# ktncktnc/diffusion-forcing-transformer

Hardware: AMD Instinct MI355X
Metric: denoised latent frames/sec, DFoT RE10K 8f & 200f rollout @1/2/4/8 GPU (higher is better)
Workload: dtype bf16

## Files before the change

diffusion-forcing-transformer_amd/backbone.py:

```python
from __future__ import annotations

import ctypes as C
import math
from typing import Dict, Optional, Sequence, Tuple

import torch
from torch import nn

from . import capi, ops
from .engine_module import EngineModule, _Node, _get

_FOURIER_BUFFERS = ("noise_level_pos_embedding.timesteps.freqs", "noise_level_pos_embedding.timesteps.phases")


class UViTModule(EngineModule):
    _family = "uvit"

    def _new_tensor(self, name: str, shape: Tuple[int, ...]) -> torch.Tensor:
        t = torch.zeros(shape, dtype=torch.float32)
        return t if name in _FOURIER_BUFFERS else nn.Parameter(t)

    def _tensors(self) -> Dict[str, torch.Tensor]:
        return self._engine_tensors()

# ... 91 lines not shown
        c.eps = 1e-6
        if int(_get(cfg, "patch_size", 2)) != 2:
            raise ValueError("only patch_size=2 is supported")
        self._ccfg = c
        self._build_tree()
        self._cond_key = None
        self._cond_refs = None
        self._cond_gen = None
        self._cond_flag = None
        self.cond_cache_stats = {"builds": 0, "identity_hits": 0, "content_hits": 0}
        self._train_names = None
        self._trainer = None
        self._trainer_sig = None
        self.live_frames = None
        self.fresh_frames = None
        self._fresh_key = None
        self._train_stamp = 0
        self._dropout_generator: Optional[torch.Generator] = None

    def _after_reserve(self) -> None:
        self._cond_key = None

    def forward(self, x: torch.Tensor, noise_levels: torch.Tensor, external_cond: Optional[torch.Tensor] = None,
                external_cond_mask: Optional[torch.Tensor] = None) -> torch.Tensor:
        assert external_cond is not None, "External condition (camera pose) is required for U-ViT3DPose model."
        if self._op_key is None:
            self._op_key = ops.register_model(self)
        if torch.is_grad_enabled() and (x.requires_grad or any(p.requires_grad for p in self.parameters())):
            if self._train_names is None:
                self._train_names = [n for n, _ in self.named_parameters()]
# ... 130 lines not shown
            self._cond_refs = (external_cond, external_cond_mask)
            self._cond_gen = self.reserve_generation
        out = torch.empty_like(xf)
        live = self.live_frames
        if live is not None:
            if tuple(live.shape) != (b, self.temporal_length) or live.dtype != torch.uint8 or not live.is_contiguous():
                raise ValueError(f"live_frames must be a contiguous uint8 tensor of shape {(b, self.temporal_length)}")
            capi.require_device(dev, live_frames=live)
        fresh = self.fresh_frames
        if fresh is not None:
            if tuple(fresh.shape) != (b, self.temporal_length) or fresh.dtype != torch.uint8 or not fresh.is_contiguous():
                raise ValueError(f"fresh_frames must be a contiguous uint8 tensor of shape {(b, self.temporal_length)}")
            capi.require_device(dev, fresh_frames=fresh)
            if key != self._fresh_key:
                fresh = None
        capi.check(capi.lib.dfot_uvit_forward_cached_masks(self._handle, capi.ptr(xf, torch.float32, "x"),
                                                           capi.ptr(kf, torch.float32, "noise_levels"), capi.ptr(out), b,
                                                           capi.ptr(live, torch.uint8, "live_frames"),
                                                           capi.ptr(fresh, torch.uint8, "fresh_frames"), capi.stream_ptr()))
        self._fresh_key = key
        return out.to(x.dtype)
```

diffusion-forcing-transformer_amd/capi.py:

```python
from __future__ import annotations

import ctypes as C
import os

_HERE = os.path.dirname(os.path.abspath(__file__))
LIB_PATH = os.environ.get("DFOT_LIB", os.path.join(_HERE, "libdfot_hip.so"))

OK, ERR_ARG, ERR_SHAPE, ERR_HIP, ERR_STATE, ERR_NAME = range(6)


class DfotError(RuntimeError):
    def __init__(self, code: int, message: str):
        super().__init__(f"libdfot_hip error {code}: {message}")
        self.code = code


class UViTConfig(C.Structure):
    _fields_ = [
        ("channels", C.c_int32 * 4), ("emb_channels", C.c_int32), ("num_updown_blocks", C.c_int32 * 3),
        ("num_mid_blocks", C.c_int32), ("num_heads", C.c_int32), ("in_channels", C.c_int32),
        ("resolution", C.c_int32), ("max_tokens", C.c_int32), ("cond_dim", C.c_int32), ("noise_dim", C.c_int32),
        ("rope_theta", C.c_float), ("eps", C.c_float),
    ]

# ... 61 lines not shown
    "dfot_uvit_num_params": (_I, [_P]),
    "dfot_uvit_param_name": (C.c_char_p, [_P, _I]),
    "dfot_uvit_param_shape": (_I, [_P, _I, C.POINTER(_L), C.POINTER(_I)]),
    "dfot_uvit_load_weight": (_I, [_P, C.c_char_p, _P, C.POINTER(_L), _I, _P]),
    "dfot_uvit_finalize": (_I, [_P, _P]),
    "dfot_uvit_reserve": (_I, [_P, _I]),
    "dfot_uvit_workspace_bytes": (C.c_size_t, [_P]),
    "dfot_uvit_set_option": (_I, [_P, C.c_char_p, _I]),
    "dfot_uvit_query": (_I, [_P, C.c_char_p, C.POINTER(C.c_double)]),
    "dfot_uvit_attn_timing": (_I, [_P, C.POINTER(C.c_double), C.POINTER(_L)]),
    "dfot_uvit_forward": (_I, [_P, _P, _P, _P, _P, _P, _I, _P]),
    "dfot_uvit_set_conditions": (_I, [_P, _P, _P, _I, _P]),
    "dfot_uvit_forward_cached": (_I, [_P, _P, _P, _P, _I, _P]),
    "dfot_uvit_forward_cached_live": (_I, [_P, _P, _P, _P, _I, _P, _P]),
    "dfot_uvit_forward_cached_masks": (_I, [_P, _P, _P, _P, _I, _P, _P, _P]),
    "dfot_uvit_read_tap": (_I, [_P, C.c_char_p, _P, C.c_size_t, _P]),
    "dfot_uvit3d_create": (_I, [C.POINTER(UViT3DConfig), C.POINTER(_P)]),
    "dfot_uvit3d_config_bytes": (_L, []),
    "dfot_uvit3d_forward": (_I, [_P, _P, _P, _P, _P, _P, _I, _P]),
    "dfot_uvit3d_forward_live": (_I, [_P, _P, _P, _P, _P, _P, _I, _P, _P]),
    "dfot_op_gn_film_silu": (_I, [_P, _P, _P, _P, _P, _P, _P, _P, _I, _I, _I, _I, _P]),
    "dfot_op_rms_film": (_I, [_P, _P, _P, _P, _P, _P, _L, _I, _I, _I, _F, _P]),
    "dfot_dit_create": (_I, [C.POINTER(DiTConfig), C.POINTER(_P)]),
    "dfot_dit_create_f": (_I, [C.POINTER(DiTConfigF), C.POINTER(_P)]),
    "dfot_dit_destroy": (_I, [_P]),
    "dfot_dit_num_params": (_I, [_P]),
    "dfot_dit_param_name": (C.c_char_p, [_P, _I]),
    "dfot_dit_param_shape": (_I, [_P, _I, C.POINTER(_L), C.POINTER(_I)]),
    "dfot_dit_load_weight": (_I, [_P, C.c_char_p, _P, C.POINTER(_L), _I, _P]),
    "dfot_dit_finalize": (_I, [_P, _P]),
# ... 244 lines not shown
```

diffusion-forcing-transformer_amd/csrc/kernels.h:

```cpp
#pragma once
#include "common.h"

namespace dfot {

int launch_noise_emb(const float* k, const float* freqs, const float* phases, const float* w1, const float* b1,
                     const float* w2, const float* b2, float* hidden, float* out, int bt, int ndim, int e, hipStream_t s);
int launch_uvit3d_emb(const float* k, const float* freqs, const float* phases, const float* w1, const float* b1, const float* w2,
                      const float* b2, const float* cond, const uint8_t* cond_mask, const float* a_w1, const float* a_b1,
                      const float* a_w2, const float* a_b2, float* out, int bt, int ndim, int cdim, int e, int tokens, hipStream_t s);
int launch_embed_input(const float* x, const float* w, const float* b, float* out, int bt, int res, int cin, int c0,
                       hipStream_t s);
int launch_cond_repack(const float* cond, bf16* a, int bt, int res, int cdim, int kpad, hipStream_t s);
int launch_emb_pyramid(const bf16* emb0, bf16* emb1, bf16* emb2, bf16* emb3, int bt, int r0, int e, hipStream_t s);
int launch_project_output(const float* x0, const float* w, const float* b, float* out, int bt, int res, int c0, int cout,
                          hipStream_t s, const uint8_t* live = nullptr);
int launch_gn_partial_f32(const float* x, float* partial, int bt, int pixels, int c, hipStream_t s);
int launch_gn_partial_bf16(const bf16* x, float* partial, int bt, int pixels, int c, hipStream_t s);
int launch_gn_finalize(const float* partial, float* stats, int bt, int nblk, int pixels, int c, float eps, hipStream_t s);
int gn_partial_blocks(int pixels);
int launch_gn_apply_silu(const float* x, const float* stats, const float* gamma, const float* beta, bf16* out, int bt,
                         int pixels, int c, hipStream_t s, const uint8_t* live = nullptr);
struct FilmChunk {
  const bf16* w;
  const float* b;
// ... 15 lines not shown
                    long m, int c, int rows_per_bt, int tokens, float eps, hipStream_t s, const RmsPending* pend = nullptr);
int launch_rms_film_bf16(const bf16* x, const float* w, const bf16* fcache, const float* sv, const uint8_t* cond_mask, bf16* out,
                         long m, int c, int rows_per_bt, int tokens, float eps, hipStream_t s, const RmsPending* pend = nullptr);

int launch_pool2_bf16(const float* x, bf16* out, int bt, int h, int w, int c, hipStream_t s);
int launch_pool2_bf16_bf16in(const bf16* x, bf16* out, int bt, int h, int w, int c, hipStream_t s);
int launch_sub_bf16_bf16in(const bf16* a, const float* b, bf16* out, long n, hipStream_t s, const uint8_t* live = nullptr, long frame_elems = 0);
int launch_upsample_add_bf16(const float* t, const bf16* skip, bf16* out, int bt, int h, int w, int c, hipStream_t s, const uint8_t* live = nullptr);
int launch_gn_apply_silu_bf16in(const bf16* x, const float* stats, const float* gamma, const float* beta, bf16* out, int bt, int pixels, int c,
                                hipStream_t s, const uint8_t* live = nullptr);
int launch_embed_input_bf16(const float* x, const float* w, const float* b, bf16* out, int bt, int res, int cin, int c0, hipStream_t s);
int launch_project_output_bf16(const bf16* x0, const float* w, const float* b, float* out, int bt, int res, int c0, int cout, hipStream_t s,
                               const uint8_t* live = nullptr);
int launch_sub_bf16(const float* a, const float* b, bf16* out, long n, hipStream_t s, const uint8_t* live = nullptr, long frame_elems = 0);
int launch_upsample_add(const float* t, const float* skip, float* out, int bt, int h, int w, int c, hipStream_t s, const uint8_t* live = nullptr);
int launch_ray_encode(const float* poses, float* out, int b, int t, int res, int normalized, hipStream_t s);
int launch_hg_prepare(const float* x, const float* noise, const float* qa, const float* qb, float* x_in, int batch,
                      int nfe, int tokens, long f, hipStream_t s);
int launch_ddim_compose(const float* x, const float* x_in, const float* v, const float* sa, const float* s1,
                        const float* an, const float* cn, const float* keep, const float* weight, const uint8_t* gen,
                        float* x_next, int batch, int nfe, int tokens, long f, bool weight_per_token, hipStream_t s);
int launch_ddim_noise(const float* noise, const float* sigma, const float* weight, const uint8_t* gen, float* x_next, int batch, int nfe,
                      int tokens, long f, bool weight_per_token, hipStream_t s);
int vloss_chunks(long f);
int launch_vloss(const float* x, const float* noise, const float* v, const float* a, const float* sg, const float* w,
                 float* x_pred, float* partial, float* loss, int batch, int tokens, long f, bool vspace, hipStream_t s);
int launch_wgrad_nt(const bf16* a, long lda, const bf16* b, long ldb, float* out, int m, int n, long rows, int slices, hipStream_t s, int img_h = 0,
                    int img_w = 0, int sdy = 0, int sdx = 0, int all_taps = 0);
struct WgradPlan {
  int form, slices;
// ... 80 lines not shown
```

diffusion-forcing-transformer_amd/csrc/kernels.hip:

```cpp
#include "kernels.h"
#include "dfot_hip.h"

namespace dfot {

typedef __attribute__((ext_vector_type(4))) float float4v;
typedef __attribute__((ext_vector_type(2))) float float2v;

__device__ __forceinline__ float wave_sum(float v) {
#pragma unroll
  for (int o = 32; o > 0; o >>= 1) v += __shfl_xor(v, o);
  return v;
}

template <bool FOURIER>
__global__ __launch_bounds__(256) void noise_mlp_kernel(const float* __restrict__ in, const float* __restrict__ freqs,
                                                        const float* __restrict__ phases, const float* __restrict__ w,
                                                        const float* __restrict__ b, float* __restrict__ out, int kdim,
                                                        int e) {
  const int lane = threadIdx.x & 63, wave = threadIdx.x >> 6;
  const int row = blockIdx.x * 4 + wave;
  const int bt = blockIdx.y;
  if (row >= e) return;
  float acc = 0.f;
  for (int i = lane; i < kdim; i += 64) {
// ... 1509 lines not shown
  hipLaunchKernelGGL(equal_bits_kernel<T>, dim3(grid), dim3(EQ_BLOCK), 0, s, (const T*)a, (const T*)b, n, rest, differs);
  DFOT_CHECK_HIP(hipGetLastError());
  return DFOT_OK;
}

int launch_equal_bits(const void* a, const void* b, long bytes, int* differs, hipStream_t s) {
  DFOT_REQUIRE(differs && ((uintptr_t)differs & 3) == 0, DFOT_ERR_ARG, "equal_bits: the flag is null or not 4-byte aligned");
  DFOT_REQUIRE(bytes >= 0, DFOT_ERR_ARG, "equal_bits: negative length %ld", bytes);
  if (bytes == 0) return DFOT_OK;
  DFOT_REQUIRE(a && b, DFOT_ERR_ARG, "equal_bits: null buffer");
  const uintptr_t al = (uintptr_t)a | (uintptr_t)b;
  if ((al & 15) == 0) return launch_equal_bits_t<uint4v>(a, b, bytes, differs, s);
  if ((al & 3) == 0) return launch_equal_bits_t<unsigned int>(a, b, bytes, differs, s);
  return launch_equal_bits_t<uint8_t>(a, b, bytes, differs, s);
}
}

extern "C" int dfot_op_equal_bits(const void* a, const void* b, int64_t bytes, int32_t* differs, void* stream) {
  return dfot::launch_equal_bits(a, b, (long)bytes, differs, (hipStream_t)stream);
}
```

diffusion-forcing-transformer_amd/csrc/uvit.hip:

```cpp
#include <algorithm>
#include <cmath>
#include <cstdarg>
#include <cstdlib>
#include <cstring>
#include <string>
#include <vector>

#include "dfot_hip.h"
#include "engine_device.h"
#include "gemm.h"
#include "kernels.h"

namespace dfot {

static thread_local char g_err[1024] = "";
void set_error(const char* fmt, ...) {
  va_list ap;
  va_start(ap, fmt);
  vsnprintf(g_err, sizeof(g_err), fmt, ap);
  va_end(ap);
}
const char* get_error() { return g_err; }

int tuning_flag(const char* name, int dflt) {
// ... 59 lines not shown
  int film_chunks = 0;
  uint8_t* cond_mask = nullptr;
  bool have_mask = false;
  int cond_batch = 0;
  int64_t cond_builds = 0;
  bf16 *acond = nullptr, *emb[4] = {nullptr, nullptr, nullptr, nullptr}, *s1 = nullptr, *hbf = nullptr,
       *cat = nullptr, *q = nullptr, *k = nullptr, *v = nullptr;
  AttnScratch attn_scratch;
  const float* pend_part = nullptr;
  float* out_part = nullptr;
  size_t out_part_elems = 0;
  const float* pend_bias = nullptr;
  int pend_lvl = 0, pend_c = 0, pend_slices = 2;
  long pend_m = 0;
  int last_batch = 0;
  const float* xin[4] = {nullptr, nullptr, nullptr, nullptr};
  bf16* XB[4] = {nullptr, nullptr, nullptr, nullptr};
  bool xin_bf[4] = {false, false, false, false};
  int gemm_variant = GEMM_AUTO;
  int attn_variant = 2;
  bool attn_force_safe = false;
  bool time_attn = false;
  std::vector<hipEvent_t> ev_start, ev_stop;
  size_t ev_used = 0;
};

namespace dfot {

static int add_res_block(dfot_uvit_s* h, const std::string& pre, int c, ResW* w) {
  const int e = h->E;
// ... 393 lines not shown
  g.A = h->s1; g.W = h->up_conv[l].w; g.M = bt * rr * rr; g.N = cout; g.K = 9 * cin; g.H = rr; g.Wd = rr; g.Cin = cin;
  g.zeros = h->zeros; g.bias = h->up_conv[l].b; g.out_f32 = h->tmp; g.ldo = cout;
  if (live && (rr * rr) % 256 == 0 && h->gemm_variant == GEMM_AUTO) g.live = live;
  if ((rc = conv_between_levels(h, g, s))) return rc;
  h->gn1_nblk = 0;
  if (!h->xin_bf[l]) {
    set_error("run_up: level %d stream is not in its bf16 buffer", l);
    return DFOT_ERR_STATE;
  }
  return launch_upsample_add_bf16(h->tmp, h->XB[l], h->XB[l], bt, rr, rr, cout, s, live);
}

}

static int forward_from_emb(dfot_uvit_s* h, const float* x, float* out, int batch, const uint8_t* live_frames, const uint8_t* fresh_frames,
                            hipStream_t s);

extern "C" {

const char* dfot_last_error(void) { return get_error(); }
int dfot_version(void) { return 1; }

int dfot_uvit_create(const dfot_uvit_config* cfg, dfot_uvit_t* out) {
  DFOT_REQUIRE(cfg && out, DFOT_ERR_ARG, "dfot_uvit_create: null argument");
  DFOT_REQUIRE(cfg->resolution % 16 == 0 && cfg->resolution >= 32, DFOT_ERR_SHAPE, "resolution %d must be a multiple of 16", cfg->resolution);
  DFOT_REQUIRE(cfg->emb_channels % 64 == 0, DFOT_ERR_SHAPE, "emb_channels %d must be a multiple of 64", cfg->emb_channels);
  DFOT_REQUIRE(cfg->in_channels <= 3 && cfg->cond_dim % 20 == 0, DFOT_ERR_SHAPE, "in_channels %d / cond_dim %d unsupported", cfg->in_channels, cfg->cond_dim);
  for (int l = 0; l < 4; ++l)
    DFOT_REQUIRE(cfg->channels[l] % 64 == 0, DFOT_ERR_SHAPE, "channels[%d]=%d must be a multiple of 64", l, cfg->channels[l]);
  DFOT_REQUIRE(cfg->channels[0] % 128 == 0 && cfg->channels[1] % 128 == 0, DFOT_ERR_SHAPE, "ResBlock channels must be multiples of 128");
  for (int l = 2; l < 4; ++l) {
// ... 165 lines not shown
      sv_off += (long)bt * 2 * c;
      return DFOT_OK;
    };
    for (int l = 0; l < 2; ++l) {
      for (ResW& w : h->down_res[l]) if ((rc = add(&w.fcache, &w.sv_off, w.w_film, w.b_film, w.c, l))) return rc;
      for (ResW& w : h->up_res[l]) if ((rc = add(&w.fcache, &w.sv_off, w.w_film, w.b_film, w.c, l))) return rc;
    }
    for (TrW& w : h->down_tr) if ((rc = add(&w.fcache, &w.sv_off, w.w_film, w.b_film, w.c, 2))) return rc;
    for (TrW& w : h->up_tr) if ((rc = add(&w.fcache, &w.sv_off, w.w_film, w.b_film, w.c, 2))) return rc;
    for (TrW& w : h->mid_tr) if ((rc = add(&w.fcache, &w.sv_off, w.w_film, w.b_film, w.c, 3))) return rc;
    if ((rc = h->alloc(&h->sv, (size_t)sv_off, true))) return rc;
    if ((rc = h->alloc(&h->film_table, table.size(), true))) return rc;
    DFOT_CHECK_HIP(hipMemcpy(h->film_table, table.data(), table.size() * sizeof(FilmChunk), hipMemcpyHostToDevice));
    h->film_chunks = (int)table.size();
    if ((rc = h->alloc(&h->cond_mask, (size_t)max_batch, true))) return rc;
    h->cond_batch = 0;
  }
  if ((rc = h->alloc(&h->cat, mc * 5, true))) return rc;
  if ((rc = h->alloc(&h->q, mc, true))) return rc;
  if ((rc = h->alloc(&h->k, mc, true))) return rc;
  if ((rc = h->alloc(&h->v, mc, true))) return rc;
  {
    const size_t e2 = bt * pix[2] * h->ch[2], e3 = bt * pix[3] * h->ch[3];
    h->out_part_elems = 3 * (e2 > e3 ? e2 : e3);
    if ((rc = h->alloc(&h->out_part, h->out_part_elems, true))) return rc;
  }
  {
    size_t need = 16;
    for (int b = 1; b <= max_batch; ++b)
      for (int l = 2; l < 4; ++l) need = std::max(need, attention_scratch_bytes(b, h->heads, h->T * h->r[l] * h->r[l], h->ch[l] / h->heads));
// ... 99 lines not shown
  h->cond_batch = batch;
  return DFOT_OK;
}

int dfot_uvit_forward_cached(dfot_uvit_t h, const float* x, const float* noise_levels, float* out, int batch, void* stream) {
  return dfot_uvit_forward_cached_live(h, x, noise_levels, out, batch, nullptr, stream);
}

int dfot_uvit_forward_cached_live(dfot_uvit_t h, const float* x, const float* noise_levels, float* out, int batch, const uint8_t* live_frames,
                                  void* stream) {
  return dfot_uvit_forward_cached_masks(h, x, noise_levels, out, batch, live_frames, nullptr, stream);
}

int dfot_uvit_forward_cached_masks(dfot_uvit_t h, const float* x, const float* noise_levels, float* out, int batch, const uint8_t* live_frames,
                                   const uint8_t* fresh_frames, void* stream) {
  DFOT_REQUIRE(h && x && noise_levels && out, DFOT_ERR_ARG, "forward: null argument");
  DFOT_REQUIRE(!fresh_frames || h->last_batch == batch, DFOT_ERR_STATE,
               "forward: frozen frames need the previous forward of this handle to have run the same batch (%d, now %d)", h->last_batch, batch);
  DFOT_REQUIRE(!fresh_frames || live_frames, DFOT_ERR_ARG, "forward: frozen frames must also be dead frames (live_frames is null)");
  DFOT_REQUIRE(!h->posefree, DFOT_ERR_STATE, "forward_cached: a pose-free handle (dfot_uvit3d_create) runs through dfot_uvit3d_forward");
  DFOT_REQUIRE(h->finalized, DFOT_ERR_STATE, "forward: weights not finalized");
  DFOT_REQUIRE(batch > 0 && batch == h->cond_batch, DFOT_ERR_STATE,
               "forward_cached: batch %d does not match the cached conditions (%d)", batch, h->cond_batch);
  hipStream_t s = (hipStream_t)stream;
  const dfot_uvit_config& c = h->cfg;
  const int bt = batch * h->T, e = h->E;
  int rc = 0;
  if ((rc = launch_noise_emb(noise_levels, h->ne_freqs, h->ne_phases, h->ne_w1, h->ne_b1, h->ne_w2, h->ne_b2, h->nhid,
                             h->nemb, bt, c.noise_dim, e, s)))
    return rc;
  return forward_from_emb(h, x, out, batch, live_frames, fresh_frames, s);
}

}

static int forward_from_emb(dfot_uvit_s* h, const float* x, float* out, int batch, const uint8_t* live_frames, const uint8_t* fresh_frames,
                            hipStream_t s) {
  const dfot_uvit_config& c = h->cfg;
  const int bt = batch * h->T, e = h->E;
  int rc = 0;
  if ((rc = launch_film_vec(h->film_table, h->film_chunks, h->nemb, h->sv, bt, e, s))) return rc;
  if ((rc = launch_embed_input_bf16(x, h->ein_w, h->ein_b, h->XB[0], bt, c.resolution, c.in_channels, h->ch[0], s))) return rc;
  h->gn1_nblk = 0;
  for (int l = 0; l < 4; ++l) h->xin[l] = h->X[l];
  h->xin_bf[0] = true;
  h->xin_bf[1] = h->xin_bf[2] = h->xin_bf[3] = false;

  if (fresh_frames && (h->gemm_variant != GEMM_AUTO || (h->r[2] * h->r[2]) % 512 != 0)) fresh_frames = nullptr;
  for (int l = 0; l < 2; ++l) {
    for (const ResW& w : h->down_res[l])
      if ((rc = run_res_block(h, w, l, bt, s, fresh_frames))) return rc;
    if ((rc = run_down(h, l, bt, s, fresh_frames))) return rc;
  }
  h->pend_bias = nullptr;
  for (const TrW& w : h->down_tr)
    if ((rc = run_tr_block(h, w, 2, batch, s))) return rc;
  if ((rc = flush_pending(h, s))) return rc;
  if ((rc = run_down(h, 2, bt, s))) return rc;
  for (const TrW& w : h->mid_tr)
    if ((rc = run_tr_block(h, w, 3, batch, s))) return rc;
  if ((rc = flush_pending(h, s))) return rc;
  if ((rc = run_up(h, 2, bt, s))) return rc;
  for (const TrW& w : h->up_tr)
    if ((rc = run_tr_block(h, w, 2, batch, s))) return rc;
  if ((rc = flush_pending(h, s))) return rc;
  for (int l = 1; l >= 0; --l) {
    if ((rc = run_up(h, l, bt, s, live_frames))) return rc;
// ... 16 lines not shown

int dfot_uvit3d_forward_live(dfot_uvit_t h, const float* x, const float* noise_levels, const float* external_cond,
                             const uint8_t* external_cond_mask, float* out, int batch, const uint8_t* live_frames, void* stream) {
  DFOT_REQUIRE(h && x && noise_levels && out, DFOT_ERR_ARG, "uvit3d_forward: null argument");
  DFOT_REQUIRE(h->posefree, DFOT_ERR_STATE, "uvit3d_forward: the handle is a pose model (dfot_uvit_create); call dfot_uvit_forward");
  DFOT_REQUIRE(h->finalized, DFOT_ERR_STATE, "uvit3d_forward: weights not finalized");
  DFOT_REQUIRE(batch > 0 && batch <= h->max_batch, DFOT_ERR_STATE, "uvit3d_forward: batch %d exceeds reserved %d", batch, h->max_batch);
  DFOT_REQUIRE(!external_cond || h->act_dim > 0, DFOT_ERR_ARG,
               "uvit3d_forward: external_cond given, but the model was built with cond_dim 0 (no external_cond_embedding)");
  hipStream_t s = (hipStream_t)stream;
  const uint8_t* mask = (external_cond && h->act_dropout) ? external_cond_mask : nullptr;
  int rc = launch_uvit3d_emb(noise_levels, h->ne_freqs, h->ne_phases, h->ne_w1, h->ne_b1, h->ne_w2, h->ne_b2, external_cond, mask, h->ac_w1,
                             h->ac_b1, h->ac_w2, h->ac_b2, h->nemb, batch * h->T, h->cfg.noise_dim, h->act_dim, h->E, h->T, s);
  if (rc) return rc;
  h->have_mask = false;
  return forward_from_emb(h, x, out, batch, live_frames, nullptr, s);
}

int dfot_uvit3d_forward(dfot_uvit_t h, const float* x, const float* noise_levels, const float* external_cond,
                        const uint8_t* external_cond_mask, float* out, int batch, void* stream) {
  return dfot_uvit3d_forward_live(h, x, noise_levels, external_cond, external_cond_mask, out, batch, nullptr, stream);
}

int dfot_op_gn_film_silu(const void* h, const float* stats, const float* gamma, const float* beta, const void* fcache, const float* sv,
                         const uint8_t* cond_mask, void* out, int bt, int pixels, int c, int tokens, void* stream) {
  DFOT_REQUIRE(h && stats && gamma && beta && sv && out, DFOT_ERR_ARG, "op_gn_film_silu: null argument");
  DFOT_REQUIRE(bt > 0 && pixels > 0 && tokens > 0 && c > 0 && c % 32 == 0, DFOT_ERR_SHAPE,
               "op_gn_film_silu: bt %d, pixels %d, tokens %d must be positive and channels %d a multiple of 32", bt, pixels, tokens, c);
  return launch_gn_film_silu((const bf16*)h, stats, gamma, beta, (const bf16*)fcache, sv, cond_mask, (bf16*)out, bt, pixels, c, tokens,
                             (hipStream_t)stream);
}
// ... 164 lines not shown
```

diffusion-forcing-transformer_amd/sampler.py:

```python
from __future__ import annotations

from dataclasses import dataclass, field
from typing import Callable, Dict, List, Optional, Tuple

import numpy as np
import torch

from . import capi, parallel
from .diffusion import DiffusionConfig, Schedule, denoising_loss, masked_mean
from .guidance import HistoryGuidance


@dataclass
class SamplerConfig:
    x_shape: Tuple[int, int, int] = (3, 256, 256)
    max_tokens: int = 8
    diffusion: DiffusionConfig = field(default_factory=DiffusionConfig)
    scheduling_matrix: str = "full_sequence"
    is_full_sequence: bool = False
    prediction_guidance: Dict = field(default_factory=lambda: {"name": "conditional"})
    interpolation_guidance: Dict = field(default_factory=lambda: {"name": "conditional"})
    keyframe_density: Optional[float] = None
    sliding_context_len: Optional[int] = None
    interpolation_max_batch_size: Optional[int] = None
# ... 22 lines not shown
        self.schedule = Schedule(cfg.diffusion)
        self.noise_fn = noise_fn or device_noise_fn(clip=cfg.diffusion.clip_noise)
        self.timesteps = cfg.diffusion.timesteps
        self.sampling_timesteps = cfg.diffusion.sampling_timesteps
        self.max_tokens = cfg.max_tokens
        self.x_shape = tuple(cfg.x_shape)
        self.trace: List[dict] = []
        self.window_forwards = 0
        self.shard_windows = False
        self.branch_parallel = False
        self._branch_split_active = False
        self.device = "cuda"
        self.dry_run = False
        self.use_graph = True
        self.skip_frozen_frames = True
        self.skip_dead_frames = True
        self.graph_replays = 0
        self.graph_captures = 0
        self._graphs: Dict[tuple, dict] = {}
        self._graphs_generation = 0
        self.attention_maps: Dict[int, dict] = {}
        if cfg.diffusion.sampling_timesteps > cfg.diffusion.timesteps:
            raise ValueError("sampling_timesteps must be <= timesteps")

    @torch.no_grad()
    def _process_conditions(self, conditions: Optional[torch.Tensor], noise_levels=None) -> Optional[torch.Tensor]:
        if conditions is None:
            return None
        if conditions.shape[-1] != 16:
            raise ValueError(f"raw camera poses must have 16 values per frame, got {conditions.shape[-1]}")
# ... 253 lines not shown
                for p_ in plans:
                    if p_.get("renoise"):
                        continue
                    lv = p_["plan"].levels.reshape(p_["bm"], horizon)
                    key = (lv == self.timesteps - 1).tobytes() + bytes([p_["nfe"]])
                    if key not in by_mask:
                        by_mask[key] = self._process_conditions(conditions.repeat_interleave(p_["nfe"], dim=0), lv)
                    p_["cond"] = by_mask[key]
            finally:
                self._interpolate_masked_poses = False
        fresh_dev = torch.from_numpy(np.concatenate([a.ravel() for a in self._fresh_flags(plans, batch_size, horizon)])).cuda()
        foff = 0
        for p_ in plans:
            p_["fresh_dev"] = fresh_dev[foff:foff + p_["bm"] * horizon].view(p_["bm"], horizon)
            foff += p_["bm"] * horizon
        xs = xs.contiguous()
        s = capi.stream_ptr
        branch_cache: Dict[tuple, tuple] = {}

        skip_dead = self.skip_dead_frames and hasattr(self.model, "live_frames")
        skip_frozen = skip_dead and self.skip_frozen_frames and hasattr(self.model, "fresh_frames")

        map_steps = set(int(i) for i in (getattr(cfg, "attention_map_steps", None) or ()))
        collect_at: Optional[int] = None
        if map_steps and not self.dry_run:
            if not hasattr(self.model, "capture_attention"):
                raise NotImplementedError(f"attention_map_steps: {type(self.model).__name__} has no attention-map capture (DiT3D backbones only)")
            self.attention_maps = {}

        def step(p_, xs, noise, tables, gen_dev, xs_next=None, live_dev=None, fresh_dev=None):
            nonlocal cond_rep, cond_nfe
            nfe, bm = p_["nfe"], p_["bm"]
            x_in = torch.empty(bm, horizon, *x_shape, device="cuda", dtype=torch.float32)
            capi.check(capi.lib.dfot_hg_prepare(capi.ptr(xs), capi.ptr(noise), capi.ptr(tables[0]), capi.ptr(tables[1]),
                                                capi.ptr(x_in), batch_size, nfe, horizon, f, s()))
            if cond_full is not None and cond_nfe != nfe:
                cond_rep = cond_full if nfe == 1 else cond_full.repeat_interleave(nfe, dim=0)
                cond_nfe = nfe
            if "cond" in p_:
                cond_rep = p_["cond"]
            lvl = tables[7] if cfg.diffusion.is_continuous else tables[7].to(torch.int32)
            world, rank = parallel.world_info()
            if nfe in split_nfe:
                hb = rank % nfe
                key = (id(cond_rep), id(p_["cmask_dev"]), hb)
# ... 7 lines not shown
                if skip_dead:
                    self.model.live_frames = gen_dev
                try:
                    v = parallel.exchange_branches(self.model(x_h, l_h, c_h, m_h), nfe)
                    self.branch_exchanges = getattr(self, "branch_exchanges", 0) + 1
                finally:
                    if skip_dead:
                        self.model.live_frames = None
            elif rg > 0:
                v = self._reconstruction_guided_v(x_in, lvl, cond_rep, p_["cmask_dev"], tables, gen_dev, rg_ctx, rg, nfe)
            else:
                if skip_dead:
                    self.model.live_frames = live_dev if live_dev is not None else p_["live_dev"]
                if skip_frozen:
                    self.model.fresh_frames = fresh_dev if fresh_dev is not None else p_["fresh_dev"]
                try:
                    v = self.model(x_in, lvl, cond_rep, p_["cmask_dev"])
                finally:
                    if skip_dead:
                        self.model.live_frames = None
                    if skip_frozen:
                        self.model.fresh_frames = None
            if collect_at is not None:
                self.attention_maps[collect_at] = {"noise_levels": lvl.clone(), **self.model.attention_maps()}
            step_noise = None
            if strict or p_["sigma"] is not None:
                step_noise = self.noise_fn("ddim", (bm, horizon, *x_shape))
            if xs_next is None:
                xs_next = torch.empty_like(xs)
            compose = capi.lib.dfot_ddim_compose_tokw if p_["tokw"] else capi.lib.dfot_ddim_compose
            capi.check(compose(capi.ptr(xs), capi.ptr(x_in), capi.ptr(v), capi.ptr(tables[2]),
                                                  capi.ptr(tables[3]), capi.ptr(tables[4]), capi.ptr(tables[5]),
                                                  capi.ptr(tables[6]), capi.ptr(p_["weights_dev"]), capi.ptr(gen_dev),
                                                  capi.ptr(xs_next), batch_size, nfe, horizon, f, s()))
            if p_["sigma"] is not None:
                nz = step_noise.to(device="cuda", dtype=torch.float32).clamp(-cfg.diffusion.clip_noise, cfg.diffusion.clip_noise).contiguous()
                capi.check(capi.lib.dfot_ddim_noise(capi.ptr(nz), capi.ptr(p_["sigma_dev"]), capi.ptr(p_["weights_dev"]), capi.ptr(gen_dev),
# ... 86 lines not shown
            if p_.get("renoise"):
                out.append(fresh)
                prev = None
                continue
            if (prev is not None and prev["bm"] == p_["bm"] and prev["nfe"] == p_["nfe"] and prev.get("cond") is p_.get("cond")
                    and ((prev["cmask"] is None and p_["cmask"] is None)
                         or (prev["cmask"] is not None and p_["cmask"] is not None and np.array_equal(prev["cmask"], p_["cmask"])))):
                a, b = prev["tables"], p_["tables"]
                same_in = (a[0] == 1) & (a[1] == 0) & (b[0] == 1) & (b[1] == 0) & (a[7] == b[7])
                untouched = np.repeat(prev["gen"].reshape(batch_size, horizon) == 0, p_["nfe"], axis=0)
                fresh = np.where(same_in & untouched, 0, 1).astype(np.uint8)
            out.append(fresh)
            prev = p_
        return out

    def _run_steps_graph(self, plans, xs, draw_noise, step, flat_dev, gens_dev, horizon):
        p0 = plans[0]
        bm, n_steps, nfe = p0["bm"], len(plans), p0["nfe"]
        need_noise = any(p_["need_noise"] for p_ in plans)
        self.model.reserve(bm)
        if hasattr(self.model, "sync_weights"):
            self.model.sync_weights()
        gen = getattr(self.model, "reserve_generation", 0)
        if gen != self._graphs_generation:
            self._graphs.clear()
            self._graphs_generation = gen
        cond_src = p0.get("cond_src")
        key = (bm, n_steps, nfe, horizon, tuple(xs.shape), need_noise, None if p0["cmask"] is None else p0["cmask"].tobytes(),
               id(self.model), None if cond_src is None else (tuple(cond_src.shape), cond_src.dtype))
        ent = self._graphs.get(key)
        if ent is None:
            ent = dict(tables=torch.empty(n_steps, 8, bm, horizon, device="cuda", dtype=torch.float32),
                       gens=torch.empty_like(gens_dev), weights=torch.empty_like(p0["weights_dev"]),
                       lives=torch.empty(n_steps, bm, horizon, device="cuda", dtype=torch.uint8),
                       fresh=torch.empty(n_steps, bm, horizon, device="cuda", dtype=torch.uint8),
                       noise=torch.empty(n_steps, bm, *xs.shape[1:], device="cuda") if need_noise else None,
                       xs=torch.empty_like(xs), out=None, graph=None,
                       cond=None if cond_src is None else torch.empty_like(cond_src),
                       cmask=p0["cmask_dev"].clone() if self._static_graph_cond and p0["cmask_dev"] is not None else None)
        ent["tables"].copy_(flat_dev.view(n_steps, 8, bm, horizon))
        ent["gens"].copy_(gens_dev)
        ent["lives"].copy_(gens_dev if nfe == 1 else gens_dev.repeat_interleave(nfe, dim=1))
        ent["fresh"].copy_(torch.stack([p_["fresh_dev"] for p_ in plans]))
        ent["weights"].copy_(p0["weights_dev"])
        if need_noise:
            for i, p_ in enumerate(plans):
                if p_["need_noise"]:
                    ent["noise"][i].copy_(draw_noise(p_))
                else:
                    ent["noise"][i].zero_()
        p_static = dict(p0, weights_dev=ent["weights"])
        if ent["cmask"] is not None:
            p_static["cmask_dev"] = ent["cmask"]
        if cond_src is not None:
            ent["cond"].copy_(cond_src)
            p_static["cond"] = ent["cond"]
        ent["xs"].copy_(step(p_static, xs, None if not need_noise else ent["noise"][0], ent["tables"][0], ent["gens"][0], live_dev=ent["lives"][0],
                            fresh_dev=ent["fresh"][0]))
        if ent["graph"] is None:
            torch.cuda.synchronize()
            graph = torch.cuda.CUDAGraph()
            with torch.cuda.graph(graph, capture_error_mode="thread_local"):
                x = ent["xs"]
                for i in range(1, n_steps):
                    x = step(p_static, x, ent["noise"][i] if need_noise else None, ent["tables"][i], ent["gens"][i], live_dev=ent["lives"][i],
                             fresh_dev=ent["fresh"][i])
                ent["out"] = x
            ent["graph"] = graph
            if len(self._graphs) >= 4:
                self._graphs.pop(next(iter(self._graphs)))
            self._graphs[key] = ent
            self.graph_captures += 1
        ent["graph"].replay()
        self.graph_replays += n_steps - 1
        return ent["out"].clone()

    @torch.no_grad()
    def _predict_sequence(self, context: torch.Tensor, length: Optional[int] = None,
                          conditions: Optional[torch.Tensor] = None, history_guidance: Optional[HistoryGuidance] = None,
                          sliding_context_len: Optional[int] = None, **_) -> Tuple[torch.Tensor, None]:
        mt = self.max_tokens
# ... 213 lines not shown
```

include/dfot_hip.h:

```cpp
#ifndef DFOT_HIP_H_
#define DFOT_HIP_H_

#include <stddef.h>
#include <stdint.h>

#ifdef __cplusplus
extern "C" {
#endif

enum {
  DFOT_OK = 0,
  DFOT_ERR_ARG = 1,
  DFOT_ERR_SHAPE = 2,
  DFOT_ERR_HIP = 3,
  DFOT_ERR_STATE = 4,
  DFOT_ERR_NAME = 5
};

typedef struct dfot_uvit_s* dfot_uvit_t;

typedef struct {
  int32_t channels[4];
  int32_t emb_channels;
  int32_t num_updown_blocks[3];
// ... 23 lines not shown
size_t dfot_uvit_workspace_bytes(dfot_uvit_t h);
int dfot_uvit_set_option(dfot_uvit_t h, const char* key, int value);
int dfot_uvit_query(dfot_uvit_t h, const char* key, double* value);
int dfot_uvit_attn_timing(dfot_uvit_t h, double* total_ms, int64_t* launches);

int dfot_uvit_forward(dfot_uvit_t h, const float* x, const float* noise_levels, const float* external_cond,
                      const uint8_t* external_cond_mask, float* out, int batch, void* stream);
int dfot_uvit_set_conditions(dfot_uvit_t h, const float* external_cond, const uint8_t* external_cond_mask, int batch,
                             void* stream);
int dfot_uvit_forward_cached(dfot_uvit_t h, const float* x, const float* noise_levels, float* out, int batch,
                             void* stream);
int dfot_uvit_forward_cached_live(dfot_uvit_t h, const float* x, const float* noise_levels, float* out, int batch,
                                  const uint8_t* live_frames, void* stream);
int dfot_uvit_forward_cached_masks(dfot_uvit_t h, const float* x, const float* noise_levels, float* out, int batch,
                                   const uint8_t* live_frames, const uint8_t* fresh_frames, void* stream);
int dfot_uvit_read_tap(dfot_uvit_t h, const char* name, float* out, size_t capacity_floats, void* stream);

typedef struct {
  int32_t channels[4];
  int32_t emb_channels;
  int32_t num_updown_blocks[3];
  int32_t num_mid_blocks;
  int32_t num_heads;
  int32_t in_channels;
  int32_t resolution;
  int32_t max_tokens;
  int32_t cond_dim;
  int32_t noise_dim;
  float rope_theta;
  float eps;
// ... 400 lines not shown
```

Before: 10.11.

## Share down-path activations across guidance branches with identical frame inputs

Adds a share_src map so that frames in later NFE (guidance) branches, whose input tables match the first branch's and are clean context, skip the convolutional down-path. Their activations are then copied from the source row after the down blocks. A new prepare kernel builds the row map and down mask, and a copy kernel duplicates the XB and HSA buffers. The intent is to avoid recomputing identical down-path work for history-guidance branches. The cost is extra small kernels and host-side numpy planning, and correctness depends on the branches being truly identical up to that point.

New measurement: 10.08. Within noise of the previous version (-0.3%).

```diff
diff --git a/diffusion-forcing-transformer_amd/backbone.py b/diffusion-forcing-transformer_amd/backbone.py
--- a/diffusion-forcing-transformer_amd/backbone.py
+++ b/diffusion-forcing-transformer_amd/backbone.py
@@ -129,6 +129,7 @@
         self._trainer_sig = None
         self.live_frames = None
         self.fresh_frames = None
+        self.share_src = None
         self._fresh_key = None
         self._train_stamp = 0
         self._dropout_generator: Optional[torch.Generator] = None
@@ -289,9 +290,15 @@
             capi.require_device(dev, fresh_frames=fresh)
             if key != self._fresh_key:
                 fresh = None
-        capi.check(capi.lib.dfot_uvit_forward_cached_masks(self._handle, capi.ptr(xf, torch.float32, "x"),
-                                                           capi.ptr(kf, torch.float32, "noise_levels"), capi.ptr(out), b,
-                                                           capi.ptr(live, torch.uint8, "live_frames"),
-                                                           capi.ptr(fresh, torch.uint8, "fresh_frames"), capi.stream_ptr()))
+        share = self.share_src
+        if share is not None:
+            if tuple(share.shape) != (b, self.temporal_length) or share.dtype != torch.int32 or not share.is_contiguous():
+                raise ValueError(f"share_src must be a contiguous int32 tensor of shape {(b, self.temporal_length)}")
+            capi.require_device(dev, share_src=share)
+        capi.check(capi.lib.dfot_uvit_forward_cached_shared(self._handle, capi.ptr(xf, torch.float32, "x"),
+                                                            capi.ptr(kf, torch.float32, "noise_levels"), capi.ptr(out), b,
+                                                            capi.ptr(live, torch.uint8, "live_frames"),
+                                                            capi.ptr(fresh, torch.uint8, "fresh_frames"),
+                                                            capi.ptr(share, torch.int32, "share_src"), capi.stream_ptr()))
         self._fresh_key = key
         return out.to(x.dtype)
diff --git a/diffusion-forcing-transformer_amd/capi.py b/diffusion-forcing-transformer_amd/capi.py
--- a/diffusion-forcing-transformer_amd/capi.py
+++ b/diffusion-forcing-transformer_amd/capi.py
@@ -99,6 +99,7 @@
     "dfot_uvit_forward_cached": (_I, [_P, _P, _P, _P, _I, _P]),
     "dfot_uvit_forward_cached_live": (_I, [_P, _P, _P, _P, _I, _P, _P]),
     "dfot_uvit_forward_cached_masks": (_I, [_P, _P, _P, _P, _I, _P, _P, _P]),
+    "dfot_uvit_forward_cached_shared": (_I, [_P, _P, _P, _P, _I, _P, _P, _P, _P]),
     "dfot_uvit_read_tap": (_I, [_P, C.c_char_p, _P, C.c_size_t, _P]),
     "dfot_uvit3d_create": (_I, [C.POINTER(UViT3DConfig), C.POINTER(_P)]),
     "dfot_uvit3d_config_bytes": (_L, []),
diff --git a/diffusion-forcing-transformer_amd/csrc/kernels.h b/diffusion-forcing-transformer_amd/csrc/kernels.h
--- a/diffusion-forcing-transformer_amd/csrc/kernels.h
+++ b/diffusion-forcing-transformer_amd/csrc/kernels.h
@@ -53,6 +53,8 @@
                                const uint8_t* live = nullptr);
 int launch_sub_bf16(const float* a, const float* b, bf16* out, long n, hipStream_t s, const uint8_t* live = nullptr, long frame_elems = 0);
 int launch_upsample_add(const float* t, const float* skip, float* out, int bt, int h, int w, int c, hipStream_t s, const uint8_t* live = nullptr);
+int launch_share_prepare(const int* share_src, const uint8_t* fresh, int* map, uint8_t* mask, int bt, hipStream_t s);
+int launch_share_rows(void* const* bufs, const long* frame_bytes, int n, const int* map, int bt, hipStream_t s);
 int launch_ray_encode(const float* poses, float* out, int b, int t, int res, int normalized, hipStream_t s);
 int launch_hg_prepare(const float* x, const float* noise, const float* qa, const float* qb, float* x_in, int batch,
                       int nfe, int tokens, long f, hipStream_t s);
diff --git a/diffusion-forcing-transformer_amd/csrc/kernels.hip b/diffusion-forcing-transformer_amd/csrc/kernels.hip
--- a/diffusion-forcing-transformer_amd/csrc/kernels.hip
+++ b/diffusion-forcing-transformer_amd/csrc/kernels.hip
@@ -1547,6 +1547,60 @@
   if ((al & 3) == 0) return launch_equal_bits_t<unsigned int>(a, b, bytes, differs, s);
   return launch_equal_bits_t<uint8_t>(a, b, bytes, differs, s);
 }
+
+__global__ void share_prepare_kernel(const int* __restrict__ share_src, const uint8_t* __restrict__ fresh, int* __restrict__ map,
+                                     uint8_t* __restrict__ mask, int bt) {
+  for (int i = threadIdx.x; i < bt; i += blockDim.x) {
+    int src = share_src[i];
+    if (src < 0 || src >= bt || src == i || share_src[src] >= 0) src = -1;
+    map[i] = src;
+    mask[i] = (uint8_t)((!fresh || fresh[i]) && src < 0);
+  }
+}
+int launch_share_prepare(const int* share_src, const uint8_t* fresh, int* map, uint8_t* mask, int bt, hipStream_t s) {
+  DFOT_REQUIRE(share_src && map && mask && bt > 0, DFOT_ERR_ARG, "share_prepare: bad argument");
+  hipLaunchKernelGGL(share_prepare_kernel, dim3(1), dim3(256), 0, s, share_src, fresh, map, mask, bt);
+  DFOT_CHECK_HIP(hipGetLastError());
+  return DFOT_OK;
+}
+
+constexpr int SHARE_BLOCK = 256, SHARE_GRID = 512;
+struct ShareBufs {
+  uint4v* p[4];
+  long frame16[4];
+};
+__global__ __launch_bounds__(SHARE_BLOCK) void share_rows_kernel(ShareBufs b, const int* __restrict__ map, int bt) {
+  uint4v* base = b.p[blockIdx.y];
+  const long n = b.frame16[blockIdx.y];
+  const long stride = (long)gridDim.x * SHARE_BLOCK;
+  for (int f = 0; f < bt; ++f) {
+    const int src = map[f];
+    if (src < 0) continue;
+    const uint4v* from = base + src * n;
+    uint4v* to = base + f * n;
+    for (long i = (long)blockIdx.x * SHARE_BLOCK + threadIdx.x; i < n; i += 2 * stride) {
+      const bool two = i + stride < n;
+      const uint4v v0 = from[i];
+      uint4v v1 = v0;
+      if (two) v1 = from[i + stride];
+      to[i] = v0;
+      if (two) to[i + stride] = v1;
+    }
+  }
+}
+int launch_share_rows(void* const* bufs, const long* frame_bytes, int n, const int* map, int bt, hipStream_t s) {
+  DFOT_REQUIRE(bufs && frame_bytes && map && n > 0 && n <= 4 && bt > 0, DFOT_ERR_ARG, "share_rows: bad argument");
+  ShareBufs b{};
+  for (int j = 0; j < n; ++j) {
+    DFOT_REQUIRE(bufs[j] && ((uintptr_t)bufs[j] & 15) == 0 && frame_bytes[j] > 0 && frame_bytes[j] % 16 == 0, DFOT_ERR_SHAPE,
+                 "share_rows: buffer %d must be 16-byte aligned with whole 16-byte vectors per frame (%ld bytes)", j, frame_bytes[j]);
+    b.p[j] = (uint4v*)bufs[j];
+    b.frame16[j] = frame_bytes[j] / 16;
+  }
+  hipLaunchKernelGGL(share_rows_kernel, dim3(SHARE_GRID, n), dim3(SHARE_BLOCK), 0, s, b, map, bt);
+  DFOT_CHECK_HIP(hipGetLastError());
+  return DFOT_OK;
+}
 }
 
 extern "C" int dfot_op_equal_bits(const void* a, const void* b, int64_t bytes, int32_t* differs, void* stream) {
diff --git a/diffusion-forcing-transformer_amd/csrc/uvit.hip b/diffusion-forcing-transformer_amd/csrc/uvit.hip
--- a/diffusion-forcing-transformer_amd/csrc/uvit.hip
+++ b/diffusion-forcing-transformer_amd/csrc/uvit.hip
@@ -97,6 +97,8 @@
   int pend_lvl = 0, pend_c = 0, pend_slices = 2;
   long pend_m = 0;
   int last_batch = 0;
+  int* share_map = nullptr;
+  uint8_t* down_mask = nullptr;
   const float* xin[4] = {nullptr, nullptr, nullptr, nullptr};
   bf16* XB[4] = {nullptr, nullptr, nullptr, nullptr};
   bool xin_bf[4] = {false, false, false, false};
@@ -520,7 +522,7 @@
 }
 
 static int forward_from_emb(dfot_uvit_s* h, const float* x, float* out, int batch, const uint8_t* live_frames, const uint8_t* fresh_frames,
-                            hipStream_t s);
+                            const int32_t* share_src, hipStream_t s);
 
 extern "C" {
 
@@ -716,6 +718,8 @@
     DFOT_CHECK_HIP(hipMemcpy(h->film_table, table.data(), table.size() * sizeof(FilmChunk), hipMemcpyHostToDevice));
     h->film_chunks = (int)table.size();
     if ((rc = h->alloc(&h->cond_mask, (size_t)max_batch, true))) return rc;
+    if ((rc = h->alloc(&h->share_map, bt, true))) return rc;
+    if ((rc = h->alloc(&h->down_mask, bt, true))) return rc;
     h->cond_batch = 0;
   }
   if ((rc = h->alloc(&h->cat, mc * 5, true))) return rc;
@@ -845,6 +849,11 @@
 
 int dfot_uvit_forward_cached_masks(dfot_uvit_t h, const float* x, const float* noise_levels, float* out, int batch, const uint8_t* live_frames,
                                    const uint8_t* fresh_frames, void* stream) {
+  return dfot_uvit_forward_cached_shared(h, x, noise_levels, out, batch, live_frames, fresh_frames, nullptr, stream);
+}
+
+int dfot_uvit_forward_cached_shared(dfot_uvit_t h, const float* x, const float* noise_levels, float* out, int batch, const uint8_t* live_frames,
+                                    const uint8_t* fresh_frames, const int32_t* share_src, void* stream) {
   DFOT_REQUIRE(h && x && noise_levels && out, DFOT_ERR_ARG, "forward: null argument");
   DFOT_REQUIRE(!fresh_frames || h->last_batch == batch, DFOT_ERR_STATE,
                "forward: frozen frames need the previous forward of this handle to have run the same batch (%d, now %d)", h->last_batch, batch);
@@ -860,13 +869,13 @@
   if ((rc = launch_noise_emb(noise_levels, h->ne_freqs, h->ne_phases, h->ne_w1, h->ne_b1, h->ne_w2, h->ne_b2, h->nhid,
                              h->nemb, bt, c.noise_dim, e, s)))
     return rc;
-  return forward_from_emb(h, x, out, batch, live_frames, fresh_frames, s);
+  return forward_from_emb(h, x, out, batch, live_frames, fresh_frames, share_src, s);
 }
 
 }
 
 static int forward_from_emb(dfot_uvit_s* h, const float* x, float* out, int batch, const uint8_t* live_frames, const uint8_t* fresh_frames,
-                            hipStream_t s) {
+                            const int32_t* share_src, hipStream_t s) {
   const dfot_uvit_config& c = h->cfg;
   const int bt = batch * h->T, e = h->E;
   int rc = 0;
@@ -877,11 +886,25 @@
   h->xin_bf[0] = true;
   h->xin_bf[1] = h->xin_bf[2] = h->xin_bf[3] = false;
 
-  if (fresh_frames && (h->gemm_variant != GEMM_AUTO || (h->r[2] * h->r[2]) % 512 != 0)) fresh_frames = nullptr;
+  if (h->gemm_variant != GEMM_AUTO || (h->r[2] * h->r[2]) % 512 != 0) fresh_frames = nullptr, share_src = nullptr;
+  const uint8_t* down = fresh_frames;
+  if (share_src) {
+    if ((rc = launch_share_prepare(share_src, fresh_frames, h->share_map, h->down_mask, bt, s))) return rc;
+    down = h->down_mask;
+  }
   for (int l = 0; l < 2; ++l) {
     for (const ResW& w : h->down_res[l])
-      if ((rc = run_res_block(h, w, l, bt, s, fresh_frames))) return rc;
-    if ((rc = run_down(h, l, bt, s, fresh_frames))) return rc;
+      if ((rc = run_res_block(h, w, l, bt, s, down))) return rc;
+    if ((rc = run_down(h, l, bt, s, down))) return rc;
+  }
+  if (share_src) {
+    void* const bufs[4] = {h->XB[0], h->XB[1], h->HSA[0], h->HSA[1]};
+    long bytes[4];
+    for (int l = 0; l < 2; ++l) {
+      bytes[l] = (long)h->r[l] * h->r[l] * h->ch[l] * (long)sizeof(bf16);
+      bytes[2 + l] = (long)h->r[l + 1] * h->r[l + 1] * h->ch[l + 1] * (long)sizeof(float);
+    }
+    if ((rc = launch_share_rows(bufs, bytes, 4, h->share_map, bt, s))) return rc;
   }
   h->pend_bias = nullptr;
   for (const TrW& w : h->down_tr)
@@ -928,7 +951,7 @@
                              h->ac_b1, h->ac_w2, h->ac_b2, h->nemb, batch * h->T, h->cfg.noise_dim, h->act_dim, h->E, h->T, s);
   if (rc) return rc;
   h->have_mask = false;
-  return forward_from_emb(h, x, out, batch, live_frames, nullptr, s);
+  return forward_from_emb(h, x, out, batch, live_frames, nullptr, nullptr, s);
 }
 
 int dfot_uvit3d_forward(dfot_uvit_t h, const float* x, const float* noise_levels, const float* external_cond,
diff --git a/diffusion-forcing-transformer_amd/sampler.py b/diffusion-forcing-transformer_amd/sampler.py
--- a/diffusion-forcing-transformer_amd/sampler.py
+++ b/diffusion-forcing-transformer_amd/sampler.py
@@ -60,6 +60,7 @@
         self.dry_run = False
         self.use_graph = True
         self.skip_frozen_frames = True
+        self.skip_shared_frames = True
         self.skip_dead_frames = True
         self.graph_replays = 0
         self.graph_captures = 0
@@ -343,12 +344,19 @@
         for p_ in plans:
             p_["fresh_dev"] = fresh_dev[foff:foff + p_["bm"] * horizon].view(p_["bm"], horizon)
             foff += p_["bm"] * horizon
+        shared = self._shared_flags(plans, batch_size, horizon)
+        share_all = torch.from_numpy(np.concatenate([a.ravel() for a in shared])).cuda() if any((a >= 0).any() for a in shared) else None
+        foff = 0
+        for p_, a in zip(plans, shared):
+            p_["share_dev"] = share_all[foff:foff + a.size].view(a.shape) if bool((a >= 0).any()) else None
+            foff += a.size
         xs = xs.contiguous()
         s = capi.stream_ptr
         branch_cache: Dict[tuple, tuple] = {}
 
         skip_dead = self.skip_dead_frames and hasattr(self.model, "live_frames")
         skip_frozen = skip_dead and self.skip_frozen_frames and hasattr(self.model, "fresh_frames")
+        skip_shared = self.skip_shared_frames and hasattr(self.model, "share_src")
 
         map_steps = set(int(i) for i in (getattr(cfg, "attention_map_steps", None) or ()))
         collect_at: Optional[int] = None
@@ -357,7 +365,7 @@
                 raise NotImplementedError(f"attention_map_steps: {type(self.model).__name__} has no attention-map capture (DiT3D backbones only)")
             self.attention_maps = {}
 
-        def step(p_, xs, noise, tables, gen_dev, xs_next=None, live_dev=None, fresh_dev=None):
+        def step(p_, xs, noise, tables, gen_dev, xs_next=None, live_dev=None, fresh_dev=None, share_dev=None):
             nonlocal cond_rep, cond_nfe
             nfe, bm = p_["nfe"], p_["bm"]
             x_in = torch.empty(bm, horizon, *x_shape, device="cuda", dtype=torch.float32)
@@ -395,6 +403,8 @@
                     self.model.live_frames = live_dev if live_dev is not None else p_["live_dev"]
                 if skip_frozen:
                     self.model.fresh_frames = fresh_dev if fresh_dev is not None else p_["fresh_dev"]
+                if skip_shared:
+                    self.model.share_src = share_dev if share_dev is not None else p_["share_dev"]
                 try:
                     v = self.model(x_in, lvl, cond_rep, p_["cmask_dev"])
                 finally:
@@ -402,6 +412,8 @@
                         self.model.live_frames = None
                     if skip_frozen:
                         self.model.fresh_frames = None
+                    if skip_shared:
+                        self.model.share_src = None
             if collect_at is not None:
                 self.attention_maps[collect_at] = {"noise_levels": lvl.clone(), **self.model.attention_maps()}
             step_noise = None
@@ -518,6 +530,23 @@
             prev = p_
         return out
 
+    @staticmethod
+    def _shared_flags(plans, batch_size: int, horizon: int):
+        out = []
+        for p_ in plans:
+            bm, nfe = p_["bm"], p_["nfe"]
+            src = np.full((bm, horizon), -1, np.int32)
+            if not p_.get("renoise") and nfe > 1 and p_.get("cond") is None:
+                t, cm = p_["tables"], p_["cmask"]
+                for r in range(bm):
+                    r0 = r - r % nfe
+                    if r == r0 or (cm is not None and bool(cm[r]) != bool(cm[r0])):
+                        continue
+                    same = (t[0, r] == t[0, r0]) & (t[1, r] == 0) & (t[1, r0] == 0) & (t[7, r] == t[7, r0])
+                    src[r] = np.where(same, r0 * horizon + np.arange(horizon), -1)
+            out.append(src)
+        return out
+
     def _run_steps_graph(self, plans, xs, draw_noise, step, flat_dev, gens_dev, horizon):
         p0 = plans[0]
         bm, n_steps, nfe = p0["bm"], len(plans), p0["nfe"]
@@ -530,14 +559,16 @@
             self._graphs.clear()
             self._graphs_generation = gen
         cond_src = p0.get("cond_src")
+        sharing = any(p_.get("share_dev") is not None for p_ in plans)
         key = (bm, n_steps, nfe, horizon, tuple(xs.shape), need_noise, None if p0["cmask"] is None else p0["cmask"].tobytes(),
-               id(self.model), None if cond_src is None else (tuple(cond_src.shape), cond_src.dtype))
+               id(self.model), None if cond_src is None else (tuple(cond_src.shape), cond_src.dtype), sharing)
         ent = self._graphs.get(key)
         if ent is None:
             ent = dict(tables=torch.empty(n_steps, 8, bm, horizon, device="cuda", dtype=torch.float32),
                        gens=torch.empty_like(gens_dev), weights=torch.empty_like(p0["weights_dev"]),
                        lives=torch.empty(n_steps, bm, horizon, device="cuda", dtype=torch.uint8),
                        fresh=torch.empty(n_steps, bm, horizon, device="cuda", dtype=torch.uint8),
+                       share=torch.empty(n_steps, bm, horizon, device="cuda", dtype=torch.int32) if sharing else None,
                        noise=torch.empty(n_steps, bm, *xs.shape[1:], device="cuda") if need_noise else None,
                        xs=torch.empty_like(xs), out=None, graph=None,
                        cond=None if cond_src is None else torch.empty_like(cond_src),
@@ -546,6 +577,11 @@
         ent["gens"].copy_(gens_dev)
         ent["lives"].copy_(gens_dev if nfe == 1 else gens_dev.repeat_interleave(nfe, dim=1))
         ent["fresh"].copy_(torch.stack([p_["fresh_dev"] for p_ in plans]))
+        if sharing:
+            ent["share"].fill_(-1)
+            for i, p_ in enumerate(plans):
+                if p_["share_dev"] is not None:
+                    ent["share"][i].copy_(p_["share_dev"])
         ent["weights"].copy_(p0["weights_dev"])
         if need_noise:
             for i, p_ in enumerate(plans):
@@ -560,7 +596,7 @@
             ent["cond"].copy_(cond_src)
             p_static["cond"] = ent["cond"]
         ent["xs"].copy_(step(p_static, xs, None if not need_noise else ent["noise"][0], ent["tables"][0], ent["gens"][0], live_dev=ent["lives"][0],
-                            fresh_dev=ent["fresh"][0]))
+                            fresh_dev=ent["fresh"][0], share_dev=ent["share"][0] if sharing else None))
         if ent["graph"] is None:
             torch.cuda.synchronize()
             graph = torch.cuda.CUDAGraph()
@@ -568,7 +604,7 @@
                 x = ent["xs"]
                 for i in range(1, n_steps):
                     x = step(p_static, x, ent["noise"][i] if need_noise else None, ent["tables"][i], ent["gens"][i], live_dev=ent["lives"][i],
-                             fresh_dev=ent["fresh"][i])
+                             fresh_dev=ent["fresh"][i], share_dev=ent["share"][i] if sharing else None)
                 ent["out"] = x
             ent["graph"] = graph
             if len(self._graphs) >= 4:
diff --git a/include/dfot_hip.h b/include/dfot_hip.h
--- a/include/dfot_hip.h
+++ b/include/dfot_hip.h
@@ -61,6 +61,8 @@
                                   const uint8_t* live_frames, void* stream);
 int dfot_uvit_forward_cached_masks(dfot_uvit_t h, const float* x, const float* noise_levels, float* out, int batch,
                                    const uint8_t* live_frames, const uint8_t* fresh_frames, void* stream);
+int dfot_uvit_forward_cached_shared(dfot_uvit_t h, const float* x, const float* noise_levels, float* out, int batch,
+                                    const uint8_t* live_frames, const uint8_t* fresh_frames, const int32_t* share_src, void* stream);
 int dfot_uvit_read_tap(dfot_uvit_t h, const char* name, float* out, size_t capacity_floats, void* stream);
 
 typedef struct {
```
